# ed-fish/data-efficient-video-transformers

Measured on AMD Instinct MI355X. Metric: clips/sec fwd+bwd, B=8 T=32 3x224x224 bf16, higher is better.
Workload: dtype bf16; 1 GPU; ViViT metric shape (SURVEY 8 'M'; BASELINE configs[2]/[3] transformer): B=8/GPU, T=32, 3x224x224, patch 16, d=512, ...; global_batch=8, parallelism=dp1

## Files before the change

### data-efficient-video-transformers_amd/csrc/gemm_common.h

```cpp
#pragma once
#include "common.h"

struct GemmParams {
  const bf16* A;
  const bf16* B;
  void* C;
  int M, N, K;
  int64_t lda, ldb, ldc;
  int epilogue, out_f32, accumulate;
  const float* bias;
  const void* residual;
  int64_t ldr;
  int res_f32;
  void* aux;
  int64_t ldaux;
  float alpha;
  int k_per_split;
  float* slab;
  int tiles_n;
  int stream_out;
  int elem;
  float* colsum_slab;
  int accumulate_colsum;
  float* bn_partial;
  const int* orow;
  int res_compact;
  int pig_blocks;
  dvt_splitk_pending pig;
  unsigned cmc, cmk;
  int cH, cW, cC, cHo, cWo, ckh, ckw, csh, csw, cph, cpw;
};

__device__ __forceinline__ int swz_mn(int k) { return (k & 3) | (((k >> 3) & 1) << 2); }
template <int ROWS> __device__ __forceinline__ int swz_mn_r(int k) {
  return ROWS >= 128 ? swz_mn(k) : (((k >> 1) & 1) | (((k >> 3) & 1) << 1));
}

__device__ __forceinline__ float epi_apply(int epi, float acc, float bias, float res, float aux_in,
                                           float& aux_out) {
  switch (epi) {
    case DVT_EPI_GELU: return gelu_erf_both_f(acc + bias, aux_out);
    case DVT_EPI_RELU: return fmaxf(acc + bias, 0.f);
    case DVT_EPI_RESIDUAL: return acc + bias + res;
    case DVT_EPI_DGELU: return acc * aux_in;
    case DVT_EPI_DRELU: return aux_in > 0.f ? acc : 0.f;
    default: return acc + bias;
  }
}


__device__ __forceinline__ void splitk_reduce_f32_part(const dvt_splitk_pending& q, int64_t first, int64_t stride) {
  const int64_t nvec = q.M * q.N / 8, MN = q.M * q.N;
  if (q.cs_slab) {
    for (int64_t m = first; m < q.M; m += stride) {
      float t = 0.f;
      for (int z = 0; z < q.splits; ++z) t += q.cs_slab[(int64_t)z * q.M + m];
      q.cs_out[m] = q.cs_accumulate ? q.cs_out[m] + t : t;
    }
  }
  for (int64_t i = first; i < nvec; i += stride) {
    const int64_t e = i * 8;
    const int64_t m = e / q.N, n = e % q.N;
    float acc[8] = {0, 0, 0, 0, 0, 0, 0, 0};
    constexpr int ZB = 8;
    int z = 0;
    for (; z + ZB <= q.splits; z += ZB) {
      float v[ZB][8];
#pragma unroll
      for (int u = 0; u < ZB; ++u) load8<float>(q.slab + (int64_t)(z + u) * MN + e, v[u]);
#pragma unroll
      for (int u = 0; u < ZB; ++u)
#pragma unroll
        for (int k = 0; k < 8; ++k) acc[k] += v[u][k];
    }
    for (; z < q.splits; ++z) {
      float v[8];
      load8<float>(q.slab + (int64_t)z * MN + e, v);
#pragma unroll
      for (int k = 0; k < 8; ++k) acc[k] += v[k];
    }
    if (q.conv_taps > 0) {
      const int64_t tap = m / q.conv_cin, ci = m - tap * q.conv_cin;
      const int64_t cin_l = q.conv_cin_l > 0 ? q.conv_cin_l : q.conv_cin, cout_l = q.conv_cout_l > 0 ? q.conv_cout_l : q.N;
      if (ci < cin_l) {
#pragma unroll
        for (int k = 0; k < 8; ++k) {
          if (n + k < cout_l) {
            float* o = q.C + ((n + k) * cin_l + ci) * q.conv_taps + tap;
            *o = q.accumulate ? *o + acc[k] : acc[k];
          }
        }
      }
      continue;
    }
    float* o = q.C + m * q.ldc + n;
    if (q.accumulate) {
      float old[8];
      load8<float>(o, old);
#pragma unroll
      for (int k = 0; k < 8; ++k) acc[k] += old[k];
    }
    store8<float>(o, acc);
  }
}

__device__ __forceinline__ void epi_apply8(int epi, float (&v)[8], const float (&bias)[8],
// ... 55 lines not shown
```

### data-efficient-video-transformers_amd/csrc/gemm_small.hip

```cpp
#include "gemm_common.h"

namespace {

constexpr int SK = 256;
constexpr int STN = 64;

__device__ __attribute__((aligned(16))) unsigned int dvt_small_zero16[4] = {0u, 0u, 0u, 0u};

__device__ __forceinline__ int swz_mn64(int k) { return ((k >> 1) & 1) | (((k >> 3) & 1) << 1); }

template <bool KMAJOR, int ROWS>
__device__ __forceinline__ void dma_chunk(const bf16* __restrict__ base, int64_t ld, int mn0, int mn_lim, int k0, int k_lim,
                                          char* img, int wid, int lane, int ck = SK) {
  const int ppw = KMAJOR ? ROWS * SK * 2 / 1024 / 4 : ck * ROWS * 2 / 1024 / 4;
  const bf16* zero = reinterpret_cast<const bf16*>(dvt_small_zero16);
#pragma unroll 4
  for (int i = 0; i < ppw; ++i) {
    const int piece = wid * ppw + i;
    const bf16* src;
    if (KMAJOR) {
      const int row = piece * 2 + (lane >> 5);
      const int c = (lane & 31) ^ (row & 15);
      const int gk = k0 + c * 8, gmn = mn0 + row;
      src = (gmn < mn_lim && gk < k_lim) ? base + (int64_t)gmn * ld + gk : zero;
    } else {
      const int k = piece * 8 + (lane >> 3);
      const int cp = lane & 7;
      const int c = ((((cp >> 1) ^ swz_mn64(k)) << 1) | (cp & 1));
      const int gk = k0 + k, gmn = mn0 + c * 8;
      src = (gk < k_lim && gmn < mn_lim) ? base + (int64_t)gk * ld + gmn : zero;
    }
    dvt_dma16(src, img + piece * 1024);
  }
}

template <typename E, bool KMAJOR>
__device__ __forceinline__ typename Elem16<E>::v8 sfrag(const char* img, int base, int kk, int g, int li) {
  typedef typename Elem16<E>::v8 V8;
  if (KMAJOR) {
    const int row = base + li;
    const int c = kk * 4 + g;
    return *reinterpret_cast<const V8*>(img + row * (SK * 2) + ((c ^ (row & 15)) << 4));
  } else {
    const int q = li >> 2, pp = li & 3;
    const int u = base >> 4;
    typename Elem16<E>::v4 half[2];
#pragma unroll
    for (int hf = 0; hf < 2; ++hf) {
      const int k = kk * 32 + 8 * g + 4 * hf + q;
      half[hf] = Elem16<E>::tr_read(img + k * 128 + ((u ^ swz_mn64(k)) << 5) + 8 * pp);
    }
    return __builtin_shufflevector(half[0], half[1], 0, 1, 2, 3, 4, 5, 6, 7);
  }
}

template <int N> __device__ __forceinline__ void swait_vm() {
  if (N == 0) asm volatile("s_waitcnt vmcnt(0)" ::: "memory");
  else if (N == 12) asm volatile("s_waitcnt vmcnt(12)" ::: "memory");
  else if (N == 16) asm volatile("s_waitcnt vmcnt(16)" ::: "memory");
  else asm volatile("s_waitcnt vmcnt(0)" ::: "memory");
}

template <typename E, bool A_KMAJOR, bool B_KMAJOR, int TM>
__device__ __forceinline__ void gemm_small_tile(const GemmParams& p, const int bid, const int nblk, char* smem) {
  static_assert(A_KMAJOR || TM == 64, "an mn-major A panel is 64 wide");
  typedef typename Elem16<E>::v8 V8;
  constexpr int WM = TM / 32, WNC = 4 / WM, WCOLS = STN / WNC, NU = WCOLS / 16;
  constexpr int kA = TM * SK * 2, kB = STN * SK * 2, kStage = kA + kB;
  constexpr int kPPC = (kA + kB) / 1024 / 4;
  const int tid = threadIdx.x, lane = tid & 63;
  const int wid = __builtin_amdgcn_readfirstlane(tid >> 6);
  const int wm = wid / WNC, wn = wid % WNC;
  const int g = lane >> 4, li = lane & 15;
  int rt, ct;
  {
    const int tiles_m = nblk / p.tiles_n;
    if ((p.tiles_n & 7) == 0) {
      const int j = bid >> 3;
      ct = (bid & 7) + 8 * (j / tiles_m);
      rt = j % tiles_m;
    } else {
      rt = bid / p.tiles_n;
      ct = bid % p.tiles_n;
    }
  }
  const int m0 = rt * TM, n0 = ct * STN;
  const int ck = (!A_KMAJOR && !B_KMAJOR && p.K <= 512) ? ((p.K + 31) & ~31) : SK;
  const int nch = (p.K + ck - 1) / ck;
  const int boff = (!A_KMAJOR && !B_KMAJOR) ? ck * 128 : kA;

  f32x4 acc[NU][2];
#pragma unroll
  for (int u = 0; u < NU; ++u)
#pragma unroll
    for (int t = 0; t < 2; ++t) acc[u][t] = f32x4{0.f, 0.f, 0.f, 0.f};

  auto issue = [&](int ch) {
    char* st = smem + (ch & 1) * kStage;
    dma_chunk<A_KMAJOR, TM>(p.A, p.lda, m0, p.M, ch * ck, p.K, st, wid, lane, ck);
    dma_chunk<B_KMAJOR, STN>(p.B, p.ldb, n0, p.N, ch * ck, p.K, st + boff, wid, lane, ck);
  };
  typedef typename Elem16<E>::v4 V4;
  const bool want_ld = p.epilogue == DVT_EPI_RESIDUAL || p.epilogue == DVT_EPI_DGELU || p.epilogue == DVT_EPI_DRELU;
  const bool want_old = p.out_f32 && p.accumulate;
  f32x4 pre_bias[NU], pre_old[2][NU];
  f32x4 pre_ld[2][NU];
#pragma unroll
  for (int u = 0; u < NU; ++u) {
    const int n = min(n0 + wn * WCOLS + u * 16 + 4 * g, p.N - 4);
    pre_bias[u] = p.bias ? *reinterpret_cast<const f32x4*>(p.bias + n) : f32x4{0.f, 0.f, 0.f, 0.f};
#pragma unroll
    for (int t = 0; t < 2; ++t) {
      const int m = min(m0 + wm * 32 + t * 16 + li, p.M - 1);
      pre_ld[t][u] = f32x4{0.f, 0.f, 0.f, 0.f};
      pre_old[t][u] = f32x4{0.f, 0.f, 0.f, 0.f};
      if (want_ld && p.epilogue == DVT_EPI_RESIDUAL && p.res_f32) {
        pre_ld[t][u] = *reinterpret_cast<const f32x4*>((const float*)p.residual + (int64_t)m * p.ldr + n);
      } else if (want_ld) {
        const E* src = p.epilogue == DVT_EPI_RESIDUAL ? (const E*)p.residual + (int64_t)m * p.ldr + n
                                                      : (const E*)p.aux + (int64_t)m * p.ldaux + n;
        const V4 h = *reinterpret_cast<const V4*>(src);
#pragma unroll
        for (int r = 0; r < 4; ++r) pre_ld[t][u][r] = (float)h[r];
      }
      if (want_old) pre_old[t][u] = *reinterpret_cast<const f32x4*>((const float*)p.C + (int64_t)m * p.ldc + n);
    }
  }
  issue(0);
  if (nch > 1) issue(1);

  const bool do_cs = !A_KMAJOR && p.colsum_slab != nullptr && n0 == 0;
  float cs = 0.f;

  for (int ch = 0; ch < nch; ++ch) {
    if (ch + 1 < nch) swait_vm<kPPC>(); else swait_vm<0>();
    __builtin_amdgcn_s_barrier();
    const char* sa = smem + (ch & 1) * kStage;
    const char* sb = sa + boff;
    auto kstep = [&](int kk) {
      V8 af[2], bfr[NU];
#pragma unroll
      for (int t = 0; t < 2; ++t) af[t] = sfrag<E, A_KMAJOR>(sa, wm * 32 + t * 16, kk, g, li);
#pragma unroll
      for (int u = 0; u < NU; ++u) bfr[u] = sfrag<E, B_KMAJOR>(sb, wn * WCOLS + u * 16, kk, g, li);
#pragma unroll
      for (int u = 0; u < NU; ++u)
#pragma unroll
        for (int t = 0; t < 2; ++t) acc[u][t] = Elem16<E>::mma(bfr[u], af[t], acc[u][t]);
    };
    if (ck == SK) {
#pragma unroll
      for (int kk = 0; kk < SK / 32; ++kk) kstep(kk);
    } else {
#pragma unroll 4
      for (int kk = 0; kk < ck / 32; ++kk) kstep(kk);
    }
    if (do_cs && tid < TM) {
#pragma unroll 8
      for (int k = 0; k < ck; ++k)
        cs += (float)*reinterpret_cast<const E*>(sa + k * 128 + (((tid >> 4) ^ swz_mn64(k)) << 5) + (tid & 15) * 2);
    }
    if (ch + 2 < nch) {
      __builtin_amdgcn_s_barrier();
      issue(ch + 2);
    }
  }
  if (do_cs && tid < TM && m0 + tid < p.M) {
    float* o = p.colsum_slab + m0 + tid;
    *o = p.accumulate_colsum ? *o + cs : cs;
  }

  float v[2][NU][4], pre[2][NU][4];
#pragma unroll
  for (int t = 0; t < 2; ++t)
#pragma unroll
    for (int u = 0; u < NU; ++u)
#pragma unroll
      for (int r = 0; r < 4; ++r) {
        v[t][u][r] = acc[u][t][r] * p.alpha;
        pre[t][u][r] = 0.f;
      }
#define DVT_SMALL_EPI(EXPR)                                  \
  _Pragma("unroll") for (int t = 0; t < 2; ++t)              \
  _Pragma("unroll") for (int u = 0; u < NU; ++u)             \
  _Pragma("unroll") for (int r = 0; r < 4; ++r) {            \
    const float bi = pre_bias[u][r], ld = pre_ld[t][u][r]; \
    float& x = v[t][u][r];                                   \
    (void)bi; (void)ld;                                      \
    EXPR;                                                    \
  }
  switch (p.epilogue) {
    case DVT_EPI_GELU: DVT_SMALL_EPI(x = gelu_erf_both_f(x + bi, pre[t][u][r])) break;
    case DVT_EPI_RELU: DVT_SMALL_EPI(x = fmaxf(x + bi, 0.f)) break;
    case DVT_EPI_RESIDUAL: DVT_SMALL_EPI(x = x + bi + ld) break;
    case DVT_EPI_DGELU: DVT_SMALL_EPI(x *= ld) break;
    case DVT_EPI_DRELU: DVT_SMALL_EPI(x = ld > 0.f ? x : 0.f) break;
    default: DVT_SMALL_EPI(x += bi) break;
  }
#undef DVT_SMALL_EPI
  const bool save_pre = p.epilogue == DVT_EPI_GELU && p.aux != nullptr;
#pragma unroll
  for (int t = 0; t < 2; ++t) {
    const int m = m0 + wm * 32 + t * 16 + li;
#pragma unroll
    for (int u = 0; u < NU; ++u) {
      const int n = n0 + wn * WCOLS + u * 16 + 4 * g;
      if (m >= p.M || n >= p.N) continue;
      if (save_pre) {
        V4 o;
#pragma unroll
        for (int r = 0; r < 4; ++r) o[r] = (E)pre[t][u][r];
        *reinterpret_cast<V4*>((E*)p.aux + (int64_t)m * p.ldaux + n) = o;
      }
      if (p.out_f32) {
        float* o = (float*)p.C + (int64_t)m * p.ldc + n;
        f32x4 w = {v[t][u][0], v[t][u][1], v[t][u][2], v[t][u][3]};
        if (p.accumulate) w += pre_old[t][u];
        *reinterpret_cast<f32x4*>(o) = w;
      } else {
        V4 o;
#pragma unroll
        for (int r = 0; r < 4; ++r) o[r] = (E)v[t][u][r];
        *reinterpret_cast<V4*>((E*)p.C + (int64_t)m * p.ldc + n) = o;
      }
    }
  }
}

template <typename E, bool A_KMAJOR, bool B_KMAJOR, int TM>
__global__ __launch_bounds__(256) void gemm_small_kernel(const GemmParams p) {
  extern __shared__ __attribute__((aligned(16))) char smem[];
  gemm_small_tile<E, A_KMAJOR, B_KMAJOR, TM>(p, blockIdx.x, gridDim.x, smem);
}

template <typename E, int TM2>
__global__ __launch_bounds__(256) void gemm_small_pair_kernel(const GemmParams pw, const GemmParams pd, const int nblk_w) {
  extern __shared__ __attribute__((aligned(16))) char smem[];
  if ((int)blockIdx.x < nblk_w) gemm_small_tile<E, false, false, 64>(pw, blockIdx.x, nblk_w, smem);
  else gemm_small_tile<E, true, false, TM2>(pd, blockIdx.x - nblk_w, gridDim.x - nblk_w, smem);
}

template <typename E, int TM2>
int launch_small_pair(const GemmParams& pw_in, const GemmParams& pd_in, hipStream_t st) {
  constexpr int kSmem = 2 * (64 + STN) * SK * 2;
  GemmParams pw = pw_in, pd = pd_in;
  pw.tiles_n = (int)dvt_cdiv(pw.N, STN);
  pd.tiles_n = (int)dvt_cdiv(pd.N, STN);
  static DvtLdsAttr attr_set;
    dvt_lds_attr(attr_set, (const void*)gemm_small_pair_kernel<E, TM2>, kSmem);
  const int nw = (int)(dvt_cdiv(pw.M, 64) * pw.tiles_n), nd = (int)(dvt_cdiv(pd.M, TM2) * pd.tiles_n);
  hipLaunchKernelGGL((gemm_small_pair_kernel<E, TM2>), dim3((unsigned)(nw + nd)), dim3(256), kSmem, st, pw, pd, nw);
  DVT_LAUNCH_CHECK("dvt_gemm_pair(small)");
  return DVT_OK;
}

template <typename E, bool AK, bool BK, int TM>
int launch_small(const GemmParams& pin, hipStream_t st) {
  constexpr int kSmem = 2 * (TM + STN) * SK * 2;
  static_assert(kSmem <= 160 * 1024, "LDS budget");
  GemmParams p = pin;
  p.tiles_n = (int)dvt_cdiv(p.N, STN);
  static DvtLdsAttr attr_set;
    dvt_lds_attr(attr_set, (const void*)gemm_small_kernel<E, AK, BK, TM>, kSmem);
  const dim3 grid((unsigned)(dvt_cdiv(p.M, TM) * p.tiles_n)), block(256);
  hipLaunchKernelGGL((gemm_small_kernel<E, AK, BK, TM>), grid, block, kSmem, st, p);
  DVT_LAUNCH_CHECK("dvt_gemm(small)");
  return DVT_OK;
}

template <typename E>
int launch_small_any(const GemmParams& p, bool ak, bool bk, int tm, hipStream_t st) {
  if (ak && bk) return tm == 32 ? launch_small<E, true, true, 32>(p, st) : launch_small<E, true, true, 64>(p, st);
  if (ak && !bk) return tm == 32 ? launch_small<E, true, false, 32>(p, st) : launch_small<E, true, false, 64>(p, st);
  if (!ak && !bk) return launch_small<E, false, false, 64>(p, st);
  return 1;
}

}

int dvt_gemm_small_tile(int64_t M, int64_t N, bool a_kmajor, bool b_kmajor) {
  if (!a_kmajor && b_kmajor) return 0;
  const int64_t t64 = dvt_cdiv(M, 64) * dvt_cdiv(N, STN);
  if (!a_kmajor) return 64;
  return t64 >= 128 ? 64 : 32;
}

int dvt_gemm_small_launch(const GemmParams& p, bool a_kmajor, bool b_kmajor, hipStream_t st) {
  const int tm = dvt_gemm_small_tile(p.M, p.N, a_kmajor, b_kmajor);
  if (tm == 0) return 1;
  if (p.elem == DVT_F16) return launch_small_any<f16>(p, a_kmajor, b_kmajor, tm, st);
  return launch_small_any<bf16>(p, a_kmajor, b_kmajor, tm, st);
}

int dvt_gemm_small_launch_pair(const GemmParams& pw, const GemmParams& pd, hipStream_t st) {
  if (pw.elem != pd.elem) return 1;
  const int tm2 = dvt_gemm_small_tile(pd.M, pd.N, true, false);
  if (tm2 == 0 || dvt_gemm_small_tile(pw.M, pw.N, false, false) != 64) return 1;
  if (pw.elem == DVT_F16) return tm2 == 32 ? launch_small_pair<f16, 32>(pw, pd, st) : launch_small_pair<f16, 64>(pw, pd, st);
  return tm2 == 32 ? launch_small_pair<bf16, 32>(pw, pd, st) : launch_small_pair<bf16, 64>(pw, pd, st);
}
```

### data-efficient-video-transformers_amd/ops.py

```python
from __future__ import annotations

import ctypes as C
import re
from typing import NamedTuple, Optional, Tuple

import torch

from . import _lib as L

Tensor = torch.Tensor

_DT = {torch.float32: L.F32, torch.bfloat16: L.BF16, torch.float16: L.F16}
_TORCH_DT = {L.F32: torch.float32, L.BF16: torch.bfloat16, L.F16: torch.float16}


def dt(t: Tensor) -> int:
    try:
        return _DT[t.dtype]
    except KeyError:
        raise TypeError(f"dtype {t.dtype} is not supported by libdvt_hip (float32 / bfloat16)")


def _stream() -> int:
    return torch.cuda.current_stream().cuda_stream
# ... 428 lines not shown
        d.pending = C.pointer(pending)
    if carry is not None:
        d.carry = C.pointer(carry)
    lib = L.load()
    nws = lib.dvt_gemm_workspace_bytes(C.byref(d))
    ws = _deferred_workspace(nws, A.device, pending) if defer_reduce else workspace(nws, A.device)
    d.workspace = _p(ws)
    if defer_reduce:
        pending._keep += (ws,)
    prof = _profiler
    if prof is not None:
        esz, osz = A.element_size(), out.element_size()
        nbytes = esz * (M * K + N * K) + osz * M * N * (2 if accumulate else 1)
        nbytes += esz * M * N * ((residual is not None) + (aux is not None))
        key = ("gemm", int(a_kmajor), int(b_kmajor), M, N, K, epilogue, nbytes)
        prof.begin(key, 2.0 * M * N * K)
        L.check(lib.dvt_gemm(C.byref(d), _stream()), "dvt_gemm")
        prof.end(key)
        return (out, pending) if defer_reduce else out
    L.check(lib.dvt_gemm(C.byref(d), _stream()), "dvt_gemm")
    return (out, pending) if defer_reduce else out


class GemmPlan(NamedTuple):
    kernel: str
    cfg: int = -1
    split: int = 1
    k_per_split: int = 0
    tile_m: int = 0
    reduce: str = "none"
    colsum: str = "none"
    carry: str = "none"
    a_kmajor: bool = True
    b_kmajor: bool = True
    epilogue: int = L.EPI_NONE
    out: str = "in"


def _enum_names(enum: str, prefix: str) -> Tuple[str, ...]:
    names = {v: re.fullmatch(prefix + r"(\w+)", k).group(1).lower() for k, v in L.ENUMS[enum].items()}
    return tuple(names[i] for i in range(len(names)))


GEMM_OUTS = ("in", "f32", "slab")
GEMM_KERNELS = _enum_names("dvt_gemm_kernel", "DVT_GEMM_K_")
GEMM_REDUCES = _enum_names("dvt_gemm_reduce", "DVT_GEMM_R_")
GEMM_COLSUMS = _enum_names("dvt_gemm_colsum", "DVT_GEMM_CS_")
GEMM_CARRIES = _enum_names("dvt_gemm_carry", "DVT_GEMM_CARRY_")


def _plan_tuple(q) -> GemmPlan:
    return GemmPlan(GEMM_KERNELS[q.kernel], q.cfg, q.split, q.k_per_split, q.tile_m, GEMM_REDUCES[q.reduce],
                    GEMM_COLSUMS[q.colsum], GEMM_CARRIES[q.carry], bool(q.a_kmajor), bool(q.b_kmajor), q.epilogue,
                    GEMM_OUTS[q.out_form])


def _plan_desc(A: Tensor, B: Tensor, M: int, N: int, K: int, *, defer_reduce: bool = False, carry=None, **kw):
    d, out = _gemm_desc(A, B, M, N, K, _launch=False, **kw)
    keep = [out]
    if defer_reduce:
        keep.append(L.SplitKPending())
        d.defer_reduce, d.pending = 1, C.pointer(keep[-1])
    if carry is not None:
        d.carry = C.pointer(carry)
    d.workspace = 256 if L.load().dvt_gemm_workspace_bytes(C.byref(d)) > 0 else None
    return d, keep


def gemm_plan(A: Tensor, B: Tensor, M: int, N: int, K: int, **kw) -> GemmPlan:
    d, _keep = _plan_desc(A, B, M, N, K, **kw)
    q = L.GemmPlanInfo()
    L.check(L.load().dvt_gemm_plan(C.byref(d), C.byref(q)), "dvt_gemm_plan")
    return _plan_tuple(q)


def gemm_pair_plan(wgrad: dict, dgrad: dict) -> Tuple[GemmPlan, GemmPlan]:
    wd, _kw = _plan_desc(**wgrad)
    gd, _kg = _plan_desc(**dgrad)
    qw, qg = L.GemmPlanInfo(), L.GemmPlanInfo()
    L.check(L.load().dvt_gemm_pair_plan(C.byref(wd), C.byref(gd), C.byref(qw), C.byref(qg)), "dvt_gemm_pair_plan")
    return _plan_tuple(qw), _plan_tuple(qg)


def gemm_is_launch_bound(M: int, N: int, K: int, dtype: torch.dtype, *, a_kmajor: bool = True, b_kmajor: bool = True) -> bool:
    if dtype not in (torch.bfloat16, torch.float16):
        return False
    d = L.GemmDesc()
    d.A = d.B = d.C = 16
    d.M, d.N, d.K = M, N, K
    d.lda, d.ldb, d.ldc = (K if a_kmajor else M), (K if b_kmajor else N), N
    d.a_kmajor, d.b_kmajor = int(a_kmajor), int(b_kmajor)
    d.in_dtype = d.out_dtype = _DT[dtype]
    d.alpha = 1.0
    return L.load().dvt_gemm_route(C.byref(d)) == 0


def splitk_reduce_pending(pending) -> None:
    if pending is not None and pending.valid:
        L.check(L.load().dvt_splitk_reduce_pending(C.byref(pending), _stream()), "dvt_splitk_reduce_pending")
        pending.valid = 0


def linear_fwd(x: Tensor, w: Tensor, bias: Optional[Tensor] = None, *, epilogue: int = L.EPI_NONE,
               residual: Optional[Tensor] = None, aux: Optional[Tensor] = None,
               out_dtype: Optional[torch.dtype] = None) -> Tensor:
    M, K = x.shape
    N = w.shape[0]
    assert w.shape[1] == K and x.stride(1) == 1 and w.is_contiguous()
    return gemm(x, w, M, N, K, a_kmajor=True, b_kmajor=True, lda=x.stride(0), ldb=K, epilogue=epilogue,
                bias=bias, residual=residual, aux=aux, out_dtype=out_dtype)


def linear_dgrad(dy: Tensor, w: Tensor, *, epilogue: int = L.EPI_NONE, aux: Optional[Tensor] = None,
                 carry=None) -> Tensor:
    M, N = dy.shape
    K = w.shape[1]
    assert w.shape[0] == N and dy.stride(1) == 1 and w.is_contiguous()
    out = gemm(dy, w, M, K, N, a_kmajor=True, b_kmajor=False, lda=dy.stride(0), ldb=K, epilogue=epilogue,
               aux=aux, carry=carry)
    if carry is not None:
        carry.valid = 0
    return out


def linear_wgrad(dy: Tensor, x: Tensor, *, out: Optional[Tensor] = None, accumulate: bool = False,
                 bias_out: Optional[Tensor] = None, bias_accumulate: bool = False, defer_reduce: bool = False):
    M, N = dy.shape
    K = x.shape[1]
    assert x.shape[0] == M and dy.stride(1) == 1 and x.stride(1) == 1
    return gemm(dy, x, N, K, M, a_kmajor=False, b_kmajor=False, lda=dy.stride(0), ldb=x.stride(0), out=out,
                out_dtype=torch.float32, accumulate=accumulate, colsum_out=bias_out,
                colsum_accumulate=bias_accumulate, defer_reduce=defer_reduce)


PAIR_LAUNCH = True


def linear_backward(dy: Tensor, x: Tensor, w: Tensor, *, out: Optional[Tensor] = None, accumulate: bool = False,
                    bias_out: Optional[Tensor] = None, bias_accumulate: bool = False, epilogue: int = L.EPI_NONE,
                    aux: Optional[Tensor] = None) -> Tuple[Tensor, Tensor]:
    M, N = dy.shape
    K = x.shape[1]
    assert x.shape[0] == M and dy.stride(1) == 1 and x.stride(1) == 1 and w.shape == (N, K) and w.is_contiguous()
    wd, out = _gemm_desc(dy, x, N, K, M, a_kmajor=False, b_kmajor=False, lda=dy.stride(0), ldb=x.stride(0), out=out,
                         out_dtype=torch.float32, accumulate=accumulate, colsum_out=bias_out,
                         colsum_accumulate=bias_accumulate)
    gd, _ = _gemm_desc(dy, w, M, K, N, a_kmajor=True, b_kmajor=False, lda=dy.stride(0), ldb=K, out=dy[:, :0].new_empty((0, K)),
                       epilogue=epilogue, aux=aux)
    gd.C, gd.ldc = dy.data_ptr(), K
    lib = L.load()
    if PAIR_LAUNCH and lib.dvt_gemm_pair_fused(C.byref(wd), C.byref(gd)):
        dx = torch.empty((M, K), dtype=dy.dtype, device=dy.device)
        gd.C, gd.ldc = dx.data_ptr(), K
        L.check(lib.dvt_gemm_pair(C.byref(wd), C.byref(gd), _stream()), "dvt_gemm_pair")
        return out, dx
    _, pend = linear_wgrad(dy, x, out=out, accumulate=accumulate, bias_out=bias_out, bias_accumulate=bias_accumulate,
                           defer_reduce=True)
    return out, linear_dgrad(dy, w, epilogue=epilogue, aux=aux, carry=pend)


def colsum(x: Tensor, *, out: Optional[Tensor] = None, accumulate: bool = False) -> Tensor:
    _need_cuda(x)
    M, N = x.shape
    assert x.stride(1) == 1
    if out is None:
        assert not accumulate
        out = torch.empty((N,), dtype=torch.float32, device=x.device)
    assert out.dtype == torch.float32 and out.numel() == N and out.is_contiguous()
    lib = L.load()
    ws = workspace(lib.dvt_colsum_workspace_bytes(M, N), x.device)
    L.check(lib.dvt_colsum(x.data_ptr(), x.stride(0), out.data_ptr(), _p(ws), M, N, dt(x), int(accumulate),
                           _stream()), "dvt_colsum")
    return out


def _attn_desc(q: Tensor, k: Tensor, v: Tensor, o: Tensor, lse: Tensor, scale: float, dropout=None) -> L.AttnDesc:
    for t in (q, k, v, o):
# ... 2279 lines not shown
```

### include/dvt_hip.h

```cpp
#ifndef DVT_HIP_H
#define DVT_HIP_H

#include <stddef.h>
#include <stdint.h>

#ifdef __cplusplus
extern "C" {
#endif

#define DVT_ABI_VERSION 5

typedef void* dvt_stream_t;

enum dvt_dtype { DVT_F32 = 0, DVT_BF16 = 1, DVT_F16 = 2 };

enum dvt_status {
  DVT_OK = 0,
  DVT_ERR_BAD_ARG = -1,
  DVT_ERR_UNSUPPORTED = -2,
  DVT_ERR_HIP = -3
};

int dvt_version(void);
const char* dvt_last_error(void);
// ... 115 lines not shown
  int32_t cs_accumulate;
  const float* cs_slab;
  float* cs_out;
  int32_t conv_cin, conv_taps;
  int32_t conv_cin_l, conv_cout_l;
} dvt_splitk_pending;

typedef struct dvt_gemm_desc {
  const void* A;
  const void* B;
  void* C;
  int64_t M, N, K;
  int64_t lda, ldb, ldc;
  int32_t a_kmajor, b_kmajor;
  int32_t in_dtype;
  int32_t out_dtype;
  int32_t epilogue;
  int32_t accumulate;
  const float* bias;
  const void* residual;
  int64_t ldr;
  void* aux;
  int64_t ldaux;
  float alpha;
  int32_t split_k;
  void* workspace;
  float* colsum_out;
  int32_t colsum_accumulate;
  int32_t defer_reduce;
  dvt_splitk_pending* pending;
  const dvt_splitk_pending* carry;
  int32_t residual_f32;
} dvt_gemm_desc;

size_t dvt_gemm_workspace_bytes(const dvt_gemm_desc* desc);
int dvt_gemm(const dvt_gemm_desc* desc, dvt_stream_t stream);
int dvt_gemm_route(const dvt_gemm_desc* desc);
enum dvt_gemm_kernel {
  DVT_GEMM_K_NONE = 0,
  DVT_GEMM_K_SMALL = 1,
  DVT_GEMM_K_SMALL_PAIR = 2,
  DVT_GEMM_K_DMA = 3,
  DVT_GEMM_K_DMA224 = 4,
  DVT_GEMM_K_MFMA128 = 5,
  DVT_GEMM_K_GENERIC64 = 6,
  DVT_GEMM_K_TINY_WAVE = 7,
  DVT_GEMM_K_TINY_THREAD = 8
};
enum dvt_gemm_reduce {
  DVT_GEMM_R_NONE = 0,
  DVT_GEMM_R_PLAIN = 1,
  DVT_GEMM_R_EPILOGUE = 2,
  DVT_GEMM_R_DEFERRED = 3
};
enum dvt_gemm_colsum {
  DVT_GEMM_CS_NONE = 0,
  DVT_GEMM_CS_FUSED = 1,
  DVT_GEMM_CS_ALONE = 2
};
enum dvt_gemm_carry {
  DVT_GEMM_CARRY_NONE = 0,
  DVT_GEMM_CARRY_TAIL = 1,
  DVT_GEMM_CARRY_ALONE = 2,
  DVT_GEMM_CARRY_WIDE = 3,
  DVT_GEMM_CARRY_CONV = 4
};
typedef struct dvt_gemm_plan_info {
  int32_t route;
  int32_t kernel;
  int32_t cfg;
  int32_t split;
  int32_t k_per_split;
  int32_t tile_m;
  int32_t reduce;
  int32_t colsum;
  int32_t carry;
  int32_t a_kmajor, b_kmajor, epilogue, out_form;
} dvt_gemm_plan_info;
int dvt_gemm_plan(const dvt_gemm_desc* desc, dvt_gemm_plan_info* info);
int dvt_gemm_pair_plan(const dvt_gemm_desc* wgrad, const dvt_gemm_desc* dgrad, dvt_gemm_plan_info* wgrad_info,
                       dvt_gemm_plan_info* dgrad_info);
int dvt_gemm_pair_fused(const dvt_gemm_desc* wgrad, const dvt_gemm_desc* dgrad);
int dvt_gemm_pair(const dvt_gemm_desc* wgrad, const dvt_gemm_desc* dgrad, dvt_stream_t stream);
int dvt_splitk_reduce_pending(const dvt_splitk_pending* pending, dvt_stream_t stream);

size_t dvt_colsum_workspace_bytes(int64_t M, int64_t N);
int dvt_colsum(const void* x, int64_t ldx, float* out, void* workspace, int64_t M, int64_t N,
               int dtype, int accumulate, dvt_stream_t stream);

typedef struct dvt_attn_desc {
  const void* q;
  const void* k;
  const void* v;
  void* o;
  float* lse;
  const void* d_o;
  void* dq;
  void* dk;
  void* dv;
  int64_t B, H, Lq, Lk, dh;
  int64_t q_sb, q_sh, q_sl;
  int64_t k_sb, k_sh, k_sl;
  int64_t v_sb, v_sh, v_sl;
  int64_t o_sb, o_sh, o_sl;
  float scale;
  int32_t dtype;
  void* workspace;
  float dropout_p;
  const uint64_t* rng_state;
  uint64_t rng_offset;
  int32_t bwd_two_pass;
} dvt_attn_desc;

size_t dvt_attention_bwd_workspace_bytes(const dvt_attn_desc* desc);
int dvt_attention_fwd(const dvt_attn_desc* desc, dvt_stream_t stream);
int dvt_attention_bwd(const dvt_attn_desc* desc, dvt_stream_t stream);
enum dvt_attn_family {
  DVT_ATTN_F_NONE = 0,
  DVT_ATTN_F_Q1 = 1,
  DVT_ATTN_F_RES = 2,
  DVT_ATTN_F_ONLINE = 3,
  DVT_ATTN_F_SMALL = 4,
  DVT_ATTN_F_GENERIC = 5,
  DVT_ATTN_B_Q1 = 6,
  DVT_ATTN_B_FUSED = 7,
  DVT_ATTN_B_PAIR = 8,
  DVT_ATTN_B_SMALL = 9,
  DVT_ATTN_B_GENERIC = 10
};
typedef struct dvt_attn_plan_info {
  int32_t family;
  int32_t count;
  int32_t count2;
  int32_t waves;
  int32_t waves2;
  int32_t patch;
  int32_t patch2;
  int32_t workspace;
  int64_t lds;
  int64_t lds2;
} dvt_attn_plan_info;
int dvt_attention_plan(const dvt_attn_desc* desc, int bwd, dvt_attn_plan_info* info);

typedef struct dvt_attn_cls_desc {
  const void* x;
  int64_t xs0, xs1;
  const float* gamma;
  const float* beta;
  float eps;
  int64_t S, N, d, H;
  int32_t dtype;
  const float* R;
  float* A;
  float* lse;
  float* P;
  float* mean;
  float* rstd;
  const float* dM;
  void* dx;
  float* G;
  float* dgamma;
  float* dbeta;
  int32_t accumulate_gamma, accumulate_beta;
  void* workspace;
} dvt_attn_cls_desc;

// ... 477 lines not shown
```

Measured before the change: 1442 clips/s.

## Shrink k-major small-GEMM chunks into a deeper LDS ring and size LDS per launch

For k-major A panels, the small GEMM kernel now streams K in 128-wide chunks through a 2- or 3-stage LDS ring (3 stages when the tile is 32 rows), instead of a 256-wide double buffer. Dynamic LDS is now sized per launch from K and layout rather than always at the maximum. Both changes aim to lower LDS use so more blocks fit per CU and to hide memory latency better. The paired wgrad/dgrad kernel also schedules the heavier role's blocks first. Smaller chunks mean more barriers per K, and the new vmcnt wait arithmetic has to match the number of DMA pieces in flight.

```diff
diff --git a/data-efficient-video-transformers_amd/csrc/gemm_common.h b/data-efficient-video-transformers_amd/csrc/gemm_common.h
--- a/data-efficient-video-transformers_amd/csrc/gemm_common.h
+++ b/data-efficient-video-transformers_amd/csrc/gemm_common.h
@@ -22,6 +22,7 @@
   int elem;
   float* colsum_slab;
   int accumulate_colsum;
+  int pair_first;
   float* bn_partial;
   const int* orow;
   int res_compact;
diff --git a/data-efficient-video-transformers_amd/csrc/gemm_small.hip b/data-efficient-video-transformers_amd/csrc/gemm_small.hip
--- a/data-efficient-video-transformers_amd/csrc/gemm_small.hip
+++ b/data-efficient-video-transformers_amd/csrc/gemm_small.hip
@@ -3,24 +3,33 @@
 namespace {
 
 constexpr int SK = 256;
+constexpr int RK = 128;
 constexpr int STN = 64;
+constexpr int ring_stages(int tm) { return tm == 32 ? 3 : 2; }
+
+inline int role_lds_bytes(int64_t K, bool a_kmajor, int tm) {
+  if (a_kmajor) return ring_stages(tm) * (tm + STN) * RK * 2;
+  return K <= 512 ? (int)((K + 31) & ~(int64_t)31) * 2 * STN * 2 : 2 * (64 + STN) * SK * 2;
+}
+constexpr int kSmallLdsMax = 2 * (64 + STN) * SK * 2;
 
 __device__ __attribute__((aligned(16))) unsigned int dvt_small_zero16[4] = {0u, 0u, 0u, 0u};
 
 __device__ __forceinline__ int swz_mn64(int k) { return ((k >> 1) & 1) | (((k >> 3) & 1) << 1); }
 
-template <bool KMAJOR, int ROWS>
+template <bool KMAJOR, int ROWS, int KD>
 __device__ __forceinline__ void dma_chunk(const bf16* __restrict__ base, int64_t ld, int mn0, int mn_lim, int k0, int k_lim,
                                           char* img, int wid, int lane, int ck = SK) {
-  const int ppw = KMAJOR ? ROWS * SK * 2 / 1024 / 4 : ck * ROWS * 2 / 1024 / 4;
+  const int ppw = KMAJOR ? ROWS * KD * 2 / 1024 / 4 : ck * ROWS * 2 / 1024 / 4;
+  constexpr int LPR = KD / 8;
   const bf16* zero = reinterpret_cast<const bf16*>(dvt_small_zero16);
 #pragma unroll 4
   for (int i = 0; i < ppw; ++i) {
     const int piece = wid * ppw + i;
     const bf16* src;
     if (KMAJOR) {
-      const int row = piece * 2 + (lane >> 5);
-      const int c = (lane & 31) ^ (row & 15);
+      const int row = piece * (64 / LPR) + lane / LPR;
+      const int c = (lane & (LPR - 1)) ^ (row & 15);
       const int gk = k0 + c * 8, gmn = mn0 + row;
       src = (gmn < mn_lim && gk < k_lim) ? base + (int64_t)gmn * ld + gk : zero;
     } else {
@@ -34,13 +43,13 @@
   }
 }
 
-template <typename E, bool KMAJOR>
+template <typename E, bool KMAJOR, int KD>
 __device__ __forceinline__ typename Elem16<E>::v8 sfrag(const char* img, int base, int kk, int g, int li) {
   typedef typename Elem16<E>::v8 V8;
   if (KMAJOR) {
     const int row = base + li;
     const int c = kk * 4 + g;
-    return *reinterpret_cast<const V8*>(img + row * (SK * 2) + ((c ^ (row & 15)) << 4));
+    return *reinterpret_cast<const V8*>(img + row * (KD * 2) + ((c ^ (row & 15)) << 4));
   } else {
     const int q = li >> 2, pp = li & 3;
     const int u = base >> 4;
@@ -55,10 +64,8 @@
 }
 
 template <int N> __device__ __forceinline__ void swait_vm() {
-  if (N == 0) asm volatile("s_waitcnt vmcnt(0)" ::: "memory");
-  else if (N == 12) asm volatile("s_waitcnt vmcnt(12)" ::: "memory");
-  else if (N == 16) asm volatile("s_waitcnt vmcnt(16)" ::: "memory");
-  else asm volatile("s_waitcnt vmcnt(0)" ::: "memory");
+  static_assert(N >= 0 && N < 64, "vmcnt is a 6-bit counter");
+  asm volatile("s_waitcnt vmcnt(%0)" ::"n"(N) : "memory");
 }
 
 template <typename E, bool A_KMAJOR, bool B_KMAJOR, int TM>
@@ -66,7 +73,9 @@
   static_assert(A_KMAJOR || TM == 64, "an mn-major A panel is 64 wide");
   typedef typename Elem16<E>::v8 V8;
   constexpr int WM = TM / 32, WNC = 4 / WM, WCOLS = STN / WNC, NU = WCOLS / 16;
-  constexpr int kA = TM * SK * 2, kB = STN * SK * 2, kStage = kA + kB;
+  constexpr int CK = A_KMAJOR ? RK : SK;
+  constexpr int NST = A_KMAJOR ? ring_stages(TM) : 2;
+  constexpr int kA = TM * CK * 2, kB = STN * CK * 2, kStage = kA + kB;
   constexpr int kPPC = (kA + kB) / 1024 / 4;
   const int tid = threadIdx.x, lane = tid & 63;
   const int wid = __builtin_amdgcn_readfirstlane(tid >> 6);
@@ -85,7 +94,7 @@
     }
   }
   const int m0 = rt * TM, n0 = ct * STN;
-  const int ck = (!A_KMAJOR && !B_KMAJOR && p.K <= 512) ? ((p.K + 31) & ~31) : SK;
+  const int ck = A_KMAJOR ? CK : (!B_KMAJOR && p.K <= 512) ? ((p.K + 31) & ~31) : SK;
   const int nch = (p.K + ck - 1) / ck;
   const int boff = (!A_KMAJOR && !B_KMAJOR) ? ck * 128 : kA;
 
@@ -96,9 +105,9 @@
     for (int t = 0; t < 2; ++t) acc[u][t] = f32x4{0.f, 0.f, 0.f, 0.f};
 
   auto issue = [&](int ch) {
-    char* st = smem + (ch & 1) * kStage;
-    dma_chunk<A_KMAJOR, TM>(p.A, p.lda, m0, p.M, ch * ck, p.K, st, wid, lane, ck);
-    dma_chunk<B_KMAJOR, STN>(p.B, p.ldb, n0, p.N, ch * ck, p.K, st + boff, wid, lane, ck);
+    char* st = smem + (ch % NST) * kStage;
+    dma_chunk<A_KMAJOR, TM, CK>(p.A, p.lda, m0, p.M, ch * ck, p.K, st, wid, lane, ck);
+    dma_chunk<B_KMAJOR, STN, CK>(p.B, p.ldb, n0, p.N, ch * ck, p.K, st + boff, wid, lane, ck);
   };
   typedef typename Elem16<E>::v4 V4;
   const bool want_ld = p.epilogue == DVT_EPI_RESIDUAL || p.epilogue == DVT_EPI_DGELU || p.epilogue == DVT_EPI_DRELU;
@@ -126,31 +135,35 @@
       if (want_old) pre_old[t][u] = *reinterpret_cast<const f32x4*>((const float*)p.C + (int64_t)m * p.ldc + n);
     }
   }
-  issue(0);
-  if (nch > 1) issue(1);
+#pragma unroll
+  for (int s = 0; s < NST; ++s)
+    if (s < nch) issue(s);
 
   const bool do_cs = !A_KMAJOR && p.colsum_slab != nullptr && n0 == 0;
   float cs = 0.f;
 
   for (int ch = 0; ch < nch; ++ch) {
-    if (ch + 1 < nch) swait_vm<kPPC>(); else swait_vm<0>();
+    const int ahead = min(nch - 1 - ch, NST - 1);
+    if (NST > 2 && ahead == 2) swait_vm<(NST > 2 ? 2 : 0) * kPPC>();
+    else if (ahead == 1) swait_vm<kPPC>();
+    else swait_vm<0>();
     __builtin_amdgcn_s_barrier();
-    const char* sa = smem + (ch & 1) * kStage;
+    const char* sa = smem + (ch % NST) * kStage;
     const char* sb = sa + boff;
     auto kstep = [&](int kk) {
       V8 af[2], bfr[NU];
 #pragma unroll
-      for (int t = 0; t < 2; ++t) af[t] = sfrag<E, A_KMAJOR>(sa, wm * 32 + t * 16, kk, g, li);
-#pragma unroll
-      for (int u = 0; u < NU; ++u) bfr[u] = sfrag<E, B_KMAJOR>(sb, wn * WCOLS + u * 16, kk, g, li);
+      for (int t = 0; t < 2; ++t) af[t] = sfrag<E, A_KMAJOR, CK>(sa, wm * 32 + t * 16, kk, g, li);
+#pragma unroll
+      for (int u = 0; u < NU; ++u) bfr[u] = sfrag<E, B_KMAJOR, CK>(sb, wn * WCOLS + u * 16, kk, g, li);
 #pragma unroll
       for (int u = 0; u < NU; ++u)
 #pragma unroll
         for (int t = 0; t < 2; ++t) acc[u][t] = Elem16<E>::mma(bfr[u], af[t], acc[u][t]);
     };
-    if (ck == SK) {
-#pragma unroll
-      for (int kk = 0; kk < SK / 32; ++kk) kstep(kk);
+    if (ck == CK) {
+#pragma unroll
+      for (int kk = 0; kk < CK / 32; ++kk) kstep(kk);
     } else {
 #pragma unroll 4
       for (int kk = 0; kk < ck / 32; ++kk) kstep(kk);
@@ -160,9 +173,9 @@
       for (int k = 0; k < ck; ++k)
         cs += (float)*reinterpret_cast<const E*>(sa + k * 128 + (((tid >> 4) ^ swz_mn64(k)) << 5) + (tid & 15) * 2);
     }
-    if (ch + 2 < nch) {
+    if (ch + NST < nch) {
       __builtin_amdgcn_s_barrier();
-      issue(ch + 2);
+      issue(ch + NST);
     }
   }
   if (do_cs && tid < TM && m0 + tid < p.M) {
@@ -236,34 +249,53 @@
 template <typename E, int TM2>
 __global__ __launch_bounds__(256) void gemm_small_pair_kernel(const GemmParams pw, const GemmParams pd, const int nblk_w) {
   extern __shared__ __attribute__((aligned(16))) char smem[];
-  if ((int)blockIdx.x < nblk_w) gemm_small_tile<E, false, false, 64>(pw, blockIdx.x, nblk_w, smem);
-  else gemm_small_tile<E, true, false, TM2>(pd, blockIdx.x - nblk_w, gridDim.x - nblk_w, smem);
+  const int bid = blockIdx.x, nblk_d = gridDim.x - nblk_w;
+  const bool dfirst = pd.pair_first != 0;
+  const int first = dfirst ? nblk_d : nblk_w;
+  const bool in_first = bid < first;
+  const int rid = in_first ? bid : bid - first;
+  if (in_first == dfirst) gemm_small_tile<E, true, false, TM2>(pd, rid, nblk_d, smem);
+  else gemm_small_tile<E, false, false, 64>(pw, rid, nblk_w, smem);
+}
+
+struct PairShape {
+  int nw, nd;
+  int lds;
+  int dgrad_first;
+};
+PairShape pair_shape(int64_t wM, int64_t wN, int64_t wK, int64_t dM, int64_t dN, int64_t dK, int tm2) {
+  PairShape s;
+  s.nw = (int)(dvt_cdiv(wM, 64) * dvt_cdiv(wN, STN));
+  s.nd = (int)(dvt_cdiv(dM, tm2) * dvt_cdiv(dN, STN));
+  const int lw = role_lds_bytes(wK, false, 64), ld = role_lds_bytes(dK, true, tm2);
+  s.lds = lw > ld ? lw : ld;
+  s.dgrad_first = dK * (tm2 + STN) > ((wK + 31) & ~(int64_t)31) * (64 + STN);
+  return s;
 }
 
 template <typename E, int TM2>
 int launch_small_pair(const GemmParams& pw_in, const GemmParams& pd_in, hipStream_t st) {
-  constexpr int kSmem = 2 * (64 + STN) * SK * 2;
   GemmParams pw = pw_in, pd = pd_in;
   pw.tiles_n = (int)dvt_cdiv(pw.N, STN);
   pd.tiles_n = (int)dvt_cdiv(pd.N, STN);
+  const PairShape s = pair_shape(pw.M, pw.N, pw.K, pd.M, pd.N, pd.K, TM2);
+  pd.pair_first = s.dgrad_first;
   static DvtLdsAttr attr_set;
-    dvt_lds_attr(attr_set, (const void*)gemm_small_pair_kernel<E, TM2>, kSmem);
-  const int nw = (int)(dvt_cdiv(pw.M, 64) * pw.tiles_n), nd = (int)(dvt_cdiv(pd.M, TM2) * pd.tiles_n);
-  hipLaunchKernelGGL((gemm_small_pair_kernel<E, TM2>), dim3((unsigned)(nw + nd)), dim3(256), kSmem, st, pw, pd, nw);
+    dvt_lds_attr(attr_set, (const void*)gemm_small_pair_kernel<E, TM2>, kSmallLdsMax);
+  hipLaunchKernelGGL((gemm_small_pair_kernel<E, TM2>), dim3((unsigned)(s.nw + s.nd)), dim3(256), s.lds, st, pw, pd, s.nw);
   DVT_LAUNCH_CHECK("dvt_gemm_pair(small)");
   return DVT_OK;
 }
 
 template <typename E, bool AK, bool BK, int TM>
 int launch_small(const GemmParams& pin, hipStream_t st) {
-  constexpr int kSmem = 2 * (TM + STN) * SK * 2;
-  static_assert(kSmem <= 160 * 1024, "LDS budget");
+  static_assert(kSmallLdsMax <= 160 * 1024, "LDS budget");
   GemmParams p = pin;
   p.tiles_n = (int)dvt_cdiv(p.N, STN);
   static DvtLdsAttr attr_set;
-    dvt_lds_attr(attr_set, (const void*)gemm_small_kernel<E, AK, BK, TM>, kSmem);
+    dvt_lds_attr(attr_set, (const void*)gemm_small_kernel<E, AK, BK, TM>, kSmallLdsMax);
   const dim3 grid((unsigned)(dvt_cdiv(p.M, TM) * p.tiles_n)), block(256);
-  hipLaunchKernelGGL((gemm_small_kernel<E, AK, BK, TM>), grid, block, kSmem, st, p);
+  hipLaunchKernelGGL((gemm_small_kernel<E, AK, BK, TM>), grid, block, role_lds_bytes(p.K, AK, TM), st, p);
   DVT_LAUNCH_CHECK("dvt_gemm(small)");
   return DVT_OK;
 }
@@ -292,6 +324,20 @@
   return launch_small_any<bf16>(p, a_kmajor, b_kmajor, tm, st);
 }
 
+int dvt_gemm_small_lds_bytes(int64_t M, int64_t N, int64_t K, int a_kmajor, int b_kmajor, int pair_tm, int* grid) {
+  if (M <= 0 || N <= 0 || K <= 0) return -1;
+  const int tm = dvt_gemm_small_tile(M, N, a_kmajor != 0, b_kmajor != 0);
+  if (tm == 0) return -1;
+  if (pair_tm == 0) {
+    if (grid) *grid = (int)(dvt_cdiv(M, tm) * dvt_cdiv(N, STN));
+    return role_lds_bytes(K, a_kmajor != 0, tm);
+  }
+  if (!a_kmajor || b_kmajor || pair_tm != tm) return -1;
+  const PairShape s = pair_shape(K, N, M, M, N, K, tm);
+  if (grid) *grid = s.nw + s.nd;
+  return s.lds;
+}
+
 int dvt_gemm_small_launch_pair(const GemmParams& pw, const GemmParams& pd, hipStream_t st) {
   if (pw.elem != pd.elem) return 1;
   const int tm2 = dvt_gemm_small_tile(pd.M, pd.N, true, false);
diff --git a/data-efficient-video-transformers_amd/ops.py b/data-efficient-video-transformers_amd/ops.py
--- a/data-efficient-video-transformers_amd/ops.py
+++ b/data-efficient-video-transformers_amd/ops.py
@@ -534,6 +534,15 @@
     return _plan_tuple(qw), _plan_tuple(qg)
 
 
+def gemm_pair(wgrad: dict, dgrad: dict) -> None:
+    wd, _ = _gemm_desc(**wgrad)
+    gd, _ = _gemm_desc(**dgrad)
+    lib = L.load()
+    if not lib.dvt_gemm_pair_fused(C.byref(wd), C.byref(gd)):
+        raise RuntimeError("gemm_pair: these two products are not one launch of the panel-streaming kernel")
+    L.check(lib.dvt_gemm_pair(C.byref(wd), C.byref(gd), _stream()), "dvt_gemm_pair")
+
+
 def gemm_is_launch_bound(M: int, N: int, K: int, dtype: torch.dtype, *, a_kmajor: bool = True, b_kmajor: bool = True) -> bool:
     if dtype not in (torch.bfloat16, torch.float16):
         return False
@@ -545,6 +554,13 @@
     d.in_dtype = d.out_dtype = _DT[dtype]
     d.alpha = 1.0
     return L.load().dvt_gemm_route(C.byref(d)) == 0
+
+
+def gemm_small_lds(M: int, N: int, K: int, *, a_kmajor: bool = True, b_kmajor: bool = True,
+                   pair_tm: int = 0) -> Optional[Tuple[int, int]]:
+    grid = C.c_int(0)
+    nbytes = L.load().dvt_gemm_small_lds_bytes(M, N, K, int(a_kmajor), int(b_kmajor), pair_tm, C.byref(grid))
+    return None if nbytes < 0 else (nbytes, grid.value)
 
 
 def splitk_reduce_pending(pending) -> None:
diff --git a/include/dvt_hip.h b/include/dvt_hip.h
--- a/include/dvt_hip.h
+++ b/include/dvt_hip.h
@@ -221,6 +221,7 @@
                        dvt_gemm_plan_info* dgrad_info);
 int dvt_gemm_pair_fused(const dvt_gemm_desc* wgrad, const dvt_gemm_desc* dgrad);
 int dvt_gemm_pair(const dvt_gemm_desc* wgrad, const dvt_gemm_desc* dgrad, dvt_stream_t stream);
+int dvt_gemm_small_lds_bytes(int64_t M, int64_t N, int64_t K, int a_kmajor, int b_kmajor, int pair_tm, int* grid);
 int dvt_splitk_reduce_pending(const dvt_splitk_pending* pending, dvt_stream_t stream);
 
 size_t dvt_colsum_workspace_bytes(int64_t M, int64_t N);
```

Result: no change. 1456 clips/s (median of 6 runs) (+1.0%).
